# sacs-epfl/decentralized-learning-simulator

Measured on AMD Instinct MI355X. Metric: device-resident GB/s, N-way weighted model-tensor reduce; 1/2/4/8 MI355X, higher is better.
Workload: dtype f32

## Files before the change

decentralized-learning-simulator_amd/csrc/dispatch.hpp:

```cpp
#pragma once

#include <hip/hip_runtime.h>

#include <algorithm>
#include <cmath>
#include <cstdint>
#include <cstdlib>
#include <cstring>
#include <type_traits>
#include <vector>

#include "dlsim.h"
#include "wreduce_kernels.hpp"
#include "chunk_mean_kernels.hpp"
#include "ab_env.hpp"


namespace dlsim_host __attribute__((visibility("hidden"))) {

int fail(int code, const char* fmt, ...) __attribute__((format(printf, 2, 3)));
int hip_fail(hipError_t e, const char* what);

constexpr int kVpt = 4;
constexpr size_t kBatchSmallBytes = size_t{1} << 20;
// ... 416 lines not shown
    if (nelem[t] * Op::kBytes > kMaxLaunchOutBytes) return false;
    if (use_defer<Op>(fan_in[t], nelem[t])) return false;
    if (!aligned16(outs[t])) return false;
    for (int i = 0; i < fan_in[t]; ++i)
      if (!aligned16(in[off[t] + i])) return false;
    return true;
  };
  std::vector<int> group;
  for (int t = 0; t < b; ++t) {
    if (batchable(t)) {
      group.push_back(t);
      continue;
    }
    if (nelem[t] == 0) continue;
    int rc = run<Op>(in + off[t], fan_in[t], w + off[t], outs[t], nelem[t], st, divs ? divs[t] : 1.0f);
    if (rc != DLSIM_OK) return rc;
  }
  std::vector<const void*> ins;
  std::vector<float> ws, dv;
  std::vector<void*> os;
  std::vector<size_t> ne, ioff;
  std::vector<int> fi;
  for (int t : group) {
    ioff.push_back(ins.size());
    for (int i = 0; i < fan_in[t]; ++i) {
      ins.push_back(in[off[t] + i]);
      ws.push_back(w[off[t] + i]);
    }
    os.push_back(outs[t]);
    ne.push_back(nelem[t]);
    fi.push_back(fan_in[t]);
    dv.push_back(divs ? divs[t] : 1.0f);
  }
  const int g = static_cast<int>(group.size());
  const size_t tile1 = dlsim::kBlock;
  int t0 = 0;
  while (t0 < g) {
    int t1 = t0, ptrs = 0;
    uint64_t blocks = 0;
    while (t1 < g && t1 - t0 < dlsim::kBatchMaxTasks && ptrs + fi[t1] <= dlsim::kBatchMaxPtrs &&
           blocks + ne[t1] / Op::E / tile1 + 1 < 0x7fffffffull) {
      ptrs += fi[t1];
      blocks += ne[t1] / Op::E / tile1 + 1;
      ++t1;
    }
    hipError_t e = launch_batch<Op>(fi.data(), ioff.data(), ins.data(), ws.data(), dv.data(), os.data(),
                                    ne.data(), t0, t1, st);
    if (e != hipSuccess) return hip_fail(e, "batched kernel launch");
    t0 = t1;
  }
  return DLSIM_OK;
}

struct TableLayout {
  size_t tasks_off, map_off, ptrs_off, w_off, bytes;
  uint32_t nblocks;
  int vpt;
};

inline size_t round8(size_t x) { return (x + 7) / 8 * 8; }

template <class Op>
uint32_t task_blocks(size_t nelem, int vpt) {
  const size_t tile = static_cast<size_t>(dlsim::kBlock) * vpt;
  return static_cast<uint32_t>(nelem / Op::E / tile + 1);
}

template <class Op>
bool table_layout(int b, const int* fan_in, const size_t* nelem, TableLayout* L) {
  uint64_t blocks = 0, ptrs = 0;
  L->vpt = batch_vpt<Op>(nelem, 0, b);
  for (int t = 0; t < b; ++t) {
    blocks += task_blocks<Op>(nelem[t], L->vpt);
    ptrs += static_cast<uint64_t>(fan_in[t]);
  }
  if (blocks >= 0x7fffffffull) return false;
  L->nblocks = static_cast<uint32_t>(blocks);
  L->tasks_off = round8(sizeof(dlsim::BatchTableHeader));
  L->map_off = round8(L->tasks_off + sizeof(dlsim::BatchTaskDesc) * static_cast<size_t>(b));
  L->ptrs_off = round8(L->map_off + sizeof(uint32_t) * static_cast<size_t>(blocks));
  L->w_off = round8(L->ptrs_off + sizeof(void*) * static_cast<size_t>(ptrs));
  L->bytes = round8(L->w_off + sizeof(float) * static_cast<size_t>(ptrs));
  return true;
}

template <class Op>
int table_fill(int b, const int* fan_in, const void* const* in, const float* w, void* const* outs,
               const size_t* nelem, void* h_table, size_t bytes) {
  TableLayout L;
  if (!table_layout<Op>(b, fan_in, nelem, &L)) return fail(DLSIM_E_ARG, "batch too large");
  if (bytes < L.bytes) return fail(DLSIM_E_ARG, "table buffer too small (%zu < %zu)", bytes, L.bytes);
  if (cross_task_overlap(b, fan_in, in, outs, nelem, Op::kBytes))
    return fail(DLSIM_E_ARG,
                "a task's output overlaps another task's input or output: one table launch runs all tasks "
                "concurrently (use separate calls, or dlsim_wreduce_batched, which orders them)");
  unsigned char* base = static_cast<unsigned char*>(h_table);
  std::memset(base, 0, L.bytes);
  auto* h = reinterpret_cast<dlsim::BatchTableHeader*>(base);
  auto* tasks = reinterpret_cast<dlsim::BatchTaskDesc*>(base + L.tasks_off);
  auto* map = reinterpret_cast<uint32_t*>(base + L.map_off);
  auto* ptrs = reinterpret_cast<const void**>(base + L.ptrs_off);
  auto* ws = reinterpret_cast<float*>(base + L.w_off);
  h->ntasks = static_cast<uint32_t>(b);
  h->nblocks = L.nblocks;
  h->vpt = static_cast<uint32_t>(L.vpt);
  h->tasks_off = L.tasks_off;
  h->map_off = L.map_off;
  h->ptrs_off = L.ptrs_off;
  h->w_off = L.w_off;
  uint32_t blk = static_cast<uint32_t>(b), off = 0;
  bool uniform = true;
  for (int t = 0; t < b; ++t) {
    const size_t total = nelem[t] * Op::kBytes;
    if (fan_in[t] > DLSIM_MAX_FUSED_INPUTS || total > kMaxLaunchOutBytes || !aligned16(outs[t]))
      return fail(DLSIM_E_ARG, "task %d cannot be table-batched (fan-in <= %d, 16-B aligned, < 2 GiB)", t,
                  DLSIM_MAX_FUSED_INPUTS);
    const uint32_t nb = task_blocks<Op>(nelem[t], L.vpt);
    tasks[t].out = outs[t];
    tasks[t].nvec = nelem[t] / Op::E;
    tasks[t].nelem = nelem[t];
    tasks[t].block_start = blk - 1;
    tasks[t].ptr_off = off;
    tasks[t].fan_in = static_cast<uint32_t>(fan_in[t]);
    map[t] = static_cast<uint32_t>(t);
    for (uint32_t k = 0; k + 1 < nb; ++k) map[blk + k] = static_cast<uint32_t>(t);
    for (int i = 0; i < fan_in[t]; ++i) {
      if (!aligned16(in[off + i]))
        return fail(DLSIM_E_ARG, "task %d input %d is not 16-byte aligned", t, i);
      ptrs[off + i] = in[off + i];
      ws[off + i] = w[off + i];
    }
    blk += nb - 1;
    off += static_cast<uint32_t>(fan_in[t]);
    uniform = uniform && fan_in[t] == fan_in[0];
  }
  h->uniform_fan_in = uniform ? static_cast<uint32_t>(fan_in[0]) : 0u;
  return DLSIM_OK;
}

template <class Op, int NF, int VPT>
hipError_t launch_table_nf(const void* d_table, uint32_t blocks, hipStream_t st) {
  hipLaunchKernelGGL((dlsim::k_wreduce_batch_table<Op, NF, group_size<Op>(), VPT, kNT, store_policy<Op>(),
                                                    kBatchWave<Op, VPT>>),
                     dim3(blocks), dim3(dlsim::kBlock), 0, st, static_cast<const unsigned char*>(d_table));
  return hipGetLastError();
}

template <class Op, int K, int VPT>
hipError_t launch_table_fixed(const void* d_table, int n, uint32_t blocks, hipStream_t st) {
  if constexpr (K > max_fixed_fan_in<Op>()) {
    return launch_table_nf<Op, 0, VPT>(d_table, blocks, st);
  } else {
    if (n == K) return launch_table_nf<Op, K, VPT>(d_table, blocks, st);
    return launch_table_fixed<Op, K + 1, VPT>(d_table, n, blocks, st);
  }
}

template <class Op>
int table_launch(const void* h_table, const void* d_table, hipStream_t st) {
  const auto* h = static_cast<const dlsim::BatchTableHeader*>(h_table);
  if (h->ntasks == 0) return DLSIM_OK;
  if (h->vpt != 1 && h->vpt != 4)
    return fail(DLSIM_E_ARG, "not a table written by dlsim_batch_table_fill (vectors per lane %u)", h->vpt);
  const int n = static_cast<int>(h->uniform_fan_in);
  hipError_t e;
  if (h->vpt == 1)
    e = n ? launch_table_fixed<Op, 1, 1>(d_table, n, h->nblocks, st) : launch_table_nf<Op, 0, 1>(d_table, h->nblocks, st);
  else
    e = n ? launch_table_fixed<Op, 1, 4>(d_table, n, h->nblocks, st) : launch_table_nf<Op, 0, 4>(d_table, h->nblocks, st);
  if (e != hipSuccess) return hip_fail(e, "table batch launch");
  return DLSIM_OK;
}


inline size_t chunk_mean_ilp_begin(int m, size_t n, int threads, size_t esz = 4, size_t vw = 8) {
  if (n <= 1) return 0;
  const size_t rnd = 128 / esz;
  size_t b = 0, e = n;
  if (!(static_cast<unsigned long long>(m) * n < 32768ULL || threads <= 1)) {
    const size_t tp = static_cast<size_t>(threads) < n ? static_cast<size_t>(threads) : n;
    const size_t cs = (n + tp - 1) / tp;
    for (size_t t = 0; t < tp; ++t) {
      size_t tb = t * cs;
      if (tb >= n) break;
      size_t te = tb + cs < n ? tb + cs : n;
      tb -= tb % rnd;
      if (te != n) te -= te % rnd;
      if (tb < te) {
        b = tb;
        e = te;
      }
    }
  }
  const size_t s1 = e - b;
  return b + (s1 >= vw ? s1 / (4 * vw) * (4 * vw) : s1 / 4 * 4);
}

using CmDefault = dlsim::CmShape<4, true, 8>;
using CmFewRows = dlsim::CmShape<4, true, 4>;
constexpr int kCmFewRowsMax = 6;

constexpr int kCmDeferRMax = 32, kCmDeferU = kDeferU, kCmDeferMinRows = 16;
inline bool chunk_defer_on() {
  static const bool on = [] {
    const char* e = dlsim::ab_getenv("DLSIM_CHUNK_DEFER");
    return !(e && e[0] == '0');
  }();
  return on;
}
inline int chunk_defer_min_m() {
  static const int k = [] {
    const char* e = dlsim::ab_getenv("DLSIM_CHUNK_DEFER_MIN_M");
    return e ? std::atoi(e) : kCmDeferMinRows;
  }();
  return k;
}
constexpr int kCmFixedMinM = 4, kCmFixedMaxM = 15;
inline bool chunk_defer_fixed_on() {
  static const bool on = [] {
    const char* e = dlsim::ab_getenv("DLSIM_CHUNK_DEFER_FIXED");
    return !(e && e[0] == '0');
  }();
  return on;
// ... 157 lines not shown
                         dim3(dlsim::kBlock), 0, st, s);
    }
    hipError_t e = hipGetLastError();
    if (e != hipSuccess) return hip_fail(e, "chunk mean batch launch");
    batch.clear();
    np = 0;
    tiles = 0;
    return DLSIM_OK;
  };
  for (int t = 0; t < b; ++t) {
    const size_t n = nelem[t];
    if (n == 0) continue;
    const int m = fan_in[t];
    const size_t ib = chunk_mean_ilp_begin(m, n, threads, Op::kBytes == 8 ? 8 : 4, dlsim::cm_lanes<Op>());
    const uint8_t flags = task_flags(t);
    const uint32_t head = m > dlsim::kCmMaxPtrs ? 0u : task_head(t, ib, flags);
    const size_t tb = task_blocks(ib, head);
    if (m > dlsim::kCmMaxPtrs) {
      void* d = nullptr;
      const size_t bytes = static_cast<size_t>(m) * sizeof(void*);
      hipError_t e = hipMallocAsync(&d, bytes, st);
      if (e != hipSuccess) return hip_fail(e, "chunk mean pointer table alloc");
      e = hipMemcpyAsync(d, in + off[t], bytes, hipMemcpyHostToDevice, st);
      if (e == hipSuccess) {
        hipLaunchKernelGGL((dlsim::k_chunk_mean_table<Op, CmDefault>), dim3(static_cast<unsigned>(tb)),
                           dim3(dlsim::kBlock), 0, st, static_cast<const void* const*>(d), m, outs[t], n, ib,
                           flags);
        e = hipGetLastError();
      }
      hipError_t e2 = hipFreeAsync(d, st);
      if (e != hipSuccess) return hip_fail(e, "chunk mean table launch");
      if (e2 != hipSuccess) return hip_fail(e2, "chunk mean pointer table free");
      continue;
    }
    if (static_cast<int>(batch.size()) == dlsim::kCmMaxTasks || np + m > dlsim::kCmMaxPtrs ||
        tiles + tb > 0x7fffffffu) {
      int rc = flush();
      if (rc != DLSIM_OK) return rc;
    }
    batch.push_back({t, ib, flags, head});
    np += m;
    tiles += tb;
  }
  return flush();
}

}

#define DLSIM_REDUCE_ENTRIES(X, Op)                                                                      \
  X int dlsim_host::run<Op>(const void* const*, int, const float*, void*, size_t, hipStream_t, float);  \
  X int dlsim_host::run_batched<Op>(int, const int*, const void* const*, const float*, void* const*,    \
                                    const size_t*, hipStream_t, const float*);                          \
  X bool dlsim_host::table_layout<Op>(int, const int*, const size_t*, dlsim_host::TableLayout*);        \
  X int dlsim_host::table_fill<Op>(int, const int*, const void* const*, const float*, void* const*,     \
                                   const size_t*, void*, size_t);                                       \
  X int dlsim_host::table_launch<Op>(const void*, const void*, hipStream_t);
#define DLSIM_MEAN_ENTRIES(X, Op)                                                                        \
  X int dlsim_host::run<Op>(const void* const*, int, const float*, void*, size_t, hipStream_t, float);  \
  X int dlsim_host::run_batched<Op>(int, const int*, const void* const*, const float*, void* const*,    \
                                    const size_t*, hipStream_t, const float*);                          \
  X int dlsim_host::run_chunk_mean<Op>(int, const int*, const void* const*, void* const*, const size_t*, \
                                       int, hipStream_t);
#define DLSIM_PROBE_ENTRIES(X, Op) \
  X int dlsim_host::run<Op>(const void* const*, int, const float*, void*, size_t, hipStream_t, float);
#define DLSIM_F64_ENTRIES(X, Op) \
  X int dlsim_host::run<Op>(const void* const*, int, const double*, void*, size_t, hipStream_t, float);
#define DLSIM_CHUNK_ENTRIES(X, Op)                                                                       \
  X int dlsim_host::run_chunk_mean<Op>(int, const int*, const void* const*, void* const*, const size_t*, \
                                       int, hipStream_t);

#define DLSIM_ALL_ENTRIES(X)                  \
  DLSIM_REDUCE_ENTRIES(X, dlsim::F32Exact)    \
  DLSIM_REDUCE_ENTRIES(X, dlsim::F32Fast)     \
  DLSIM_REDUCE_ENTRIES(X, dlsim::BF16Exact)   \
  DLSIM_REDUCE_ENTRIES(X, dlsim::BF16Fast)    \
  DLSIM_REDUCE_ENTRIES(X, dlsim::F16Exact)    \
  DLSIM_REDUCE_ENTRIES(X, dlsim::F16Fast)     \
  DLSIM_MEAN_ENTRIES(X, dlsim::F32Mean)       \
  DLSIM_MEAN_ENTRIES(X, dlsim::BF16Mean)      \
  DLSIM_MEAN_ENTRIES(X, dlsim::F16Mean)       \
  DLSIM_PROBE_ENTRIES(X, dlsim::XorProbe<4>)  \
  DLSIM_PROBE_ENTRIES(X, dlsim::XorProbe<2>)  \
  DLSIM_F64_ENTRIES(X, dlsim::F64Exact)       \
  DLSIM_F64_ENTRIES(X, dlsim::F64Fast)        \
  DLSIM_CHUNK_ENTRIES(X, dlsim::F64Mean)
```

decentralized-learning-simulator_amd/csrc/dlsim_abi.hip:

```cpp
#include <hip/hip_runtime.h>

#include <algorithm>
#include <cstdarg>
#include <cstdio>
#include <cstdint>
#include <cstdlib>
#include <cstring>
#include <mutex>
#include <string>
#include <thread>
#include <vector>

#include "abi_common.hpp"
#include "dispatch.hpp"
#include "fanin_checks.hpp"

#include "host_pack.hpp"

namespace dlsim_host __attribute__((visibility("hidden"))) {

template <class F>
int with_policy(int dtype, int mode, F&& f) {
  const bool fast = mode == DLSIM_FAST;
  if (dtype == DLSIM_F32) return fast ? f(dlsim::F32Fast{}) : f(dlsim::F32Exact{});
// ... 317 lines not shown
int dlsim_wreduce_tensors(const void* const* d_inputs, int n, int t, const size_t* numels,
                          const float* h_weights, void* const* d_outs, int dtype, int mode,
                          void* stream) {
  g_err.clear();
  if (t < 0) return fail(DLSIM_E_ARG, "t must be >= 0 (got %d)", t);
  if (t > 0 && (!d_inputs || !numels || !d_outs)) return fail(DLSIM_E_ARG, "null array argument");
  if (n < 1) return fail(DLSIM_E_ARG, "n must be >= 1 (got %d)", n);
  if (!h_weights) return fail(DLSIM_E_ARG, "null weights array");
  std::vector<const void*> ins(static_cast<size_t>(n) * t);
  std::vector<float> ws(static_cast<size_t>(n) * t);
  std::vector<int> fan(static_cast<size_t>(t), n);
  for (int k = 0; k < t; ++k) {
    for (int i = 0; i < n; ++i) {
      ins[static_cast<size_t>(k) * n + i] = d_inputs[static_cast<size_t>(i) * t + k];
      ws[static_cast<size_t>(k) * n + i] = h_weights[i];
    }
    int rc = check_args(&ins[static_cast<size_t>(k) * n], n, h_weights, d_outs[k], numels[k], dtype, mode);
    if (rc != DLSIM_OK) return fail(rc, "tensor %d: %s", k, g_err.c_str());
  }
  if (t == 0) return DLSIM_OK;
  hipStream_t st = static_cast<hipStream_t>(stream);
  return with_policy(dtype, mode, [&](auto op) {
    return run_batched<decltype(op)>(t, fan.data(), ins.data(), ws.data(), d_outs, numels, st);
  });
}

int dlsim_wreduce_batched(int b, const int* fan_in, const void* const* d_inputs,
                          const float* h_weights, void* const* d_outs, const size_t* n_elems,
                          int dtype, int mode, void* stream) {
  g_err.clear();
  if (b < 0) return fail(DLSIM_E_ARG, "b must be >= 0 (got %d)", b);
  if (b == 0) return DLSIM_OK;
  if (!fan_in || !d_inputs || !h_weights || !d_outs || !n_elems) return fail(DLSIM_E_ARG, "null array argument");
  size_t off = 0;
  for (int t = 0; t < b; ++t) {
    int rc = check_args(d_inputs + off, fan_in[t], h_weights + off, d_outs[t], n_elems[t], dtype, mode);
    if (rc != DLSIM_OK) return fail(rc, "task %d: %s", t, g_err.c_str());
    off += static_cast<size_t>(fan_in[t]);
  }
  hipStream_t st = static_cast<hipStream_t>(stream);
  return with_policy(dtype, mode, [&](auto op) {
    return run_batched<decltype(op)>(b, fan_in, d_inputs, h_weights, d_outs, n_elems, st);
  });
}

int dlsim_batch_table_bytes(int b, const int* fan_in, const size_t* n_elems, int dtype, size_t* bytes) {
  g_err.clear();
  if (b < 0 || (b > 0 && (!fan_in || !n_elems)) || !bytes) return fail(DLSIM_E_ARG, "bad arguments");
  if (!known_dtype(dtype)) return dtype_fail(dtype);
  for (int t = 0; t < b; ++t)
    if (fan_in[t] < 1) return fail(DLSIM_E_ARG, "task %d: fan-in must be >= 1", t);
  TableLayout L;
  const bool ok = with_policy(dtype, DLSIM_EXACT, [&](auto op) {
    return table_layout<decltype(op)>(b, fan_in, n_elems, &L) ? 1 : 0;
  }) != 0;
  if (!ok) return fail(DLSIM_E_ARG, "batch too large");
  *bytes = L.bytes;
  return DLSIM_OK;
}

int dlsim_batch_table_fill(int b, const int* fan_in, const void* const* d_inputs, const float* h_weights,
                           void* const* d_outs, const size_t* n_elems, int dtype, void* h_table,
                           size_t table_bytes) {
  g_err.clear();
  if (b < 0 || !h_table) return fail(DLSIM_E_ARG, "bad arguments");
  if (b > 0 && (!fan_in || !d_inputs || !h_weights || !d_outs || !n_elems))
    return fail(DLSIM_E_ARG, "null array argument");
  size_t off = 0;
  for (int t = 0; t < b; ++t) {
    int rc = check_args(d_inputs + off, fan_in[t], h_weights + off, d_outs[t], n_elems[t], dtype, DLSIM_EXACT);
    if (rc != DLSIM_OK) return fail(rc, "task %d: %s", t, g_err.c_str());
    off += static_cast<size_t>(fan_in[t]);
  }
  return with_policy(dtype, DLSIM_EXACT, [&](auto op) {
    return table_fill<decltype(op)>(b, fan_in, d_inputs, h_weights, d_outs, n_elems, h_table, table_bytes);
  });
}

int dlsim_batch_table_launch(const void* h_table, const void* d_table, int dtype, int mode, void* stream) {
  g_err.clear();
  if (!h_table || !d_table) return fail(DLSIM_E_ARG, "null table");
  if (!known_dtype(dtype)) return dtype_fail(dtype);
  if (mode != DLSIM_EXACT && mode != DLSIM_FAST) return fail(DLSIM_E_MODE, "unsupported mode %d", mode);
  hipStream_t st = static_cast<hipStream_t>(stream);
  return with_policy(dtype, mode, [&](auto op) { return table_launch<decltype(op)>(h_table, d_table, st); });
}

int dlsim_mean(const void* const* d_inputs, int n, void* d_out, size_t n_elems, int dtype,
               void* stream) {
  g_err.clear();
  int rc = check_args(d_inputs, n, nullptr, d_out, n_elems, dtype, DLSIM_EXACT, false);
  if (rc != DLSIM_OK) return rc;
  hipStream_t st = static_cast<hipStream_t>(stream);
  const float div = static_cast<float>(n);
  return with_mean_policy(dtype, [&](auto op) {
    return run<decltype(op)>(d_inputs, n, nullptr, d_out, n_elems, st, div);
  });
}

int dlsim_mean_batched(int b, const int* fan_in, const void* const* d_inputs, void* const* d_outs,
                       const size_t* n_elems, int dtype, void* stream) {
  g_err.clear();
  if (b < 0) return fail(DLSIM_E_ARG, "b must be >= 0 (got %d)", b);
  if (b == 0) return DLSIM_OK;
  if (!fan_in || !d_inputs || !d_outs || !n_elems) return fail(DLSIM_E_ARG, "null array argument");
  size_t off = 0;
  std::vector<float> divs(static_cast<size_t>(b));
  for (int t = 0; t < b; ++t) {
    int rc = check_args(d_inputs + off, fan_in[t], nullptr, d_outs[t], n_elems[t], dtype, DLSIM_EXACT, false);
    if (rc != DLSIM_OK) return fail(rc, "task %d: %s", t, g_err.c_str());
// ... 932 lines not shown
```

decentralized-learning-simulator_amd/csrc/wreduce_kernels.hpp:

```cpp
#pragma once

#include <hip/hip_runtime.h>
#include <stdint.h>

#include <type_traits>

#pragma clang fp contract(off)

namespace dlsim {

constexpr int kBlock = 256;

typedef uint32_t u32x4 __attribute__((ext_vector_type(4)));
typedef float f32x2 __attribute__((ext_vector_type(2)));
typedef __bf16 bf16x2 __attribute__((ext_vector_type(2)));

__device__ __forceinline__ float bf16_round(float f) {
  uint32_t u = __float_as_uint(f);
  if ((u & 0x7fffffffu) > 0x7f800000u) return __uint_as_float(0x7fc00000u);
  u += 0x7fffu + ((u >> 16) & 1u);
  return __uint_as_float(u & 0xffff0000u);
}

__device__ __forceinline__ void bf16_round2(float& a0, float& a1) {
// ... 724 lines not shown
}

struct TaskArgs {
  const BatchSlots& b;
  int off;
  float d;
  __device__ const void* ptr(int i) const { return b.p[off + i]; }
  __device__ float wt(int i) const { return b.w[off + i]; }
  __device__ float divisor() const { return d; }
};

template <class Op, int NF, int G, int VPT, int NT, int STP, bool WAVEMAP = false>
__global__ __launch_bounds__(kBlock) void k_wreduce_batch(const BatchSlots s) {
  const uint32_t bid = blockIdx.x;
  int t = 0;
  uint32_t local = 0;
  if (bid < static_cast<uint32_t>(s.ntasks)) {
    t = static_cast<int>(bid);
  } else {
    const uint32_t f = bid - static_cast<uint32_t>(s.ntasks);
    t = batch_find_task(s, f);
    local = f - s.block_start[t] + 1;
  }
  const TaskArgs a{s, static_cast<int>(s.ptr_off[t]), s.div[t]};
  const int n = NF > 0 ? NF : static_cast<int>(s.fan_in[t]);
  const size_t nvec = s.nvec[t];
  constexpr size_t kTile = static_cast<size_t>(kBlock) * VPT;
  const size_t full = nvec / kTile;
  const OutRef o = make_out<STP>(s.out[t], nvec);
  if (local == 0) {
    if (full * kTile < nvec)
      reduce_tile<Op, TaskArgs, NF, G, VPT, NT, true, STP>(a, n, o, full * kTile + threadIdx.x, nvec);
    const size_t j = nvec * Op::E + threadIdx.x;
    if (j < s.nelem[t]) fold_scalar<Op, TaskArgs>(a, n, s.out[t], j);
    return;
  }
  if constexpr (WAVEMAP) {
    const size_t lane_off = (threadIdx.x >> 6) * 64 * VPT + (threadIdx.x & 63);
    reduce_tile<Op, TaskArgs, NF, G, VPT, NT, false, STP, 64>(a, n, o, (local - 1) * kTile + lane_off, nvec);
  } else {
    reduce_tile<Op, TaskArgs, NF, G, VPT, NT, false, STP>(a, n, o, (local - 1) * kTile + threadIdx.x, nvec);
  }
}

struct BatchTableHeader {
  uint32_t ntasks;
  uint32_t nblocks;
  uint32_t uniform_fan_in;
  uint32_t vpt;
  uint64_t tasks_off;
  uint64_t map_off;
  uint64_t ptrs_off;
  uint64_t w_off;
};

struct BatchTaskDesc {
  void* out;
  uint64_t nvec;
  uint64_t nelem;
  uint32_t block_start;
  uint32_t ptr_off;
  uint32_t fan_in;
  uint32_t reserved;
};

struct TableArgs {
  const void* const* p;
  const float* w;
  __device__ const void* ptr(int i) const { return p[i]; }
  __device__ float wt(int i) const { return w[i]; }
  __device__ float divisor() const { return 1.0f; }
};

template <class Op, int NF, int G, int VPT, int NT, int STP, bool WAVEMAP = false>
__global__ __launch_bounds__(kBlock) void k_wreduce_batch_table(const unsigned char* __restrict__ table) {
  const BatchTableHeader* h = reinterpret_cast<const BatchTableHeader*>(table);
  const uint32_t* map = reinterpret_cast<const uint32_t*>(table + h->map_off);
  const uint32_t t = map[blockIdx.x];
  const BatchTaskDesc d = reinterpret_cast<const BatchTaskDesc*>(table + h->tasks_off)[t];
  const TableArgs a{reinterpret_cast<const void* const*>(table + h->ptrs_off) + d.ptr_off,
                    reinterpret_cast<const float*>(table + h->w_off) + d.ptr_off};
  const int n = NF > 0 ? NF : static_cast<int>(d.fan_in);
  const size_t nvec = d.nvec;
  constexpr size_t kTile = static_cast<size_t>(kBlock) * VPT;
  const size_t full = nvec / kTile;
  const OutRef o = make_out<STP>(d.out, nvec);
  const uint32_t local = blockIdx.x < h->ntasks ? 0u : blockIdx.x - d.block_start;
  if (local == 0) {
    if (full * kTile < nvec)
      reduce_tile<Op, TableArgs, NF, G, VPT, NT, true, STP>(a, n, o, full * kTile + threadIdx.x, nvec);
    const size_t j = nvec * Op::E + threadIdx.x;
    if (j < d.nelem) fold_scalar<Op, TableArgs>(a, n, d.out, j);
    return;
  }
  if constexpr (WAVEMAP) {
    const size_t lane_off = (threadIdx.x >> 6) * 64 * VPT + (threadIdx.x & 63);
    reduce_tile<Op, TableArgs, NF, G, VPT, NT, false, STP, 64>(a, n, o, (local - 1) * kTile + lane_off, nvec);
  } else {
    reduce_tile<Op, TableArgs, NF, G, VPT, NT, false, STP>(a, n, o, (local - 1) * kTile + threadIdx.x, nvec);
  }
}

template <int BYTES>
struct XorProbe {
  static constexpr int E = 16 / BYTES;
  static constexpr int kBytes = BYTES;
// ... 87 lines not shown
```

decentralized-learning-simulator_amd/dasklearn_amd/_native.py:

```python
from __future__ import annotations

import ctypes
import os
import threading
from typing import Optional, Sequence

import numpy as np

LIB_DIR = os.path.join(os.path.dirname(os.path.abspath(__file__)), "lib")
LIB_PATH = os.path.join(LIB_DIR, "libdlsim_hip.so")

DLSIM_F32 = 0
DLSIM_BF16 = 1
DLSIM_F16 = 2
DLSIM_F64 = 3
DLSIM_EXACT = 0
DLSIM_FAST = 1
MAX_FUSED_INPUTS = 128
DLSIM_E_ARG = -1
DLSIM_E_RCCL = -4
DLSIM_E_PEER = -5
DLSIM_E_DISAGREE = -6
DLSIM_GATHER_NONE = 0
DLSIM_GATHER_BCAST = 1
DLSIM_GATHER_ALLGATHER = 2


def ab_env(name: str, default: Optional[str] = None) -> Optional[str]:
    if os.environ.get("DLSIM_AB") != "1":
        return default
    return os.environ.get(name, default)

EXPORTS = (
    "dlsim_wreduce",
    "dlsim_wreduce_f64",
    "dlsim_wreduce_tensors",
    "dlsim_wreduce_batched",
    "dlsim_batch_table_bytes",
    "dlsim_batch_table_fill",
    "dlsim_batch_table_launch",
    "dlsim_mean",
    "dlsim_mean_batched",
    "dlsim_chunk_mean_batched",
    "dlsim_chunk_mean_ilp_begin",
    "dlsim_rccl_bind",
    "dlsim_wreduce_sharded",
    "dlsim_wreduce_sharded_f64",
    "dlsim_wreduce_mixed",
    "dlsim_sgd_step",
    "dlsim_sgd_step_tensors",
    "dlsim_sgd_momentum_step",
    "dlsim_sgd_momentum_step_tensors",
    "dlsim_robust_reduce",
    "dlsim_robust_reduce_tensors",
    "dlsim_robust_reduce_batched",
    "dlsim_robust_batch_geometry",
    "dlsim_robust_reduce_tensors_batched",
    "dlsim_pairwise_sqdist",
    "dlsim_pairwise_sqdist_tensors",
    "dlsim_pairdist_geometry",
    "dlsim_wreduce_dist",
    "dlsim_wreduce_dist_tensors",
    "dlsim_reducedist_geometry",
    "dlsim_device_alloc",
    "dlsim_device_free",
    "dlsim_pool_alloc",
    "dlsim_pool_free",
    "dlsim_pool_stats",
    "dlsim_sharded_plan_create",
    "dlsim_sharded_plan_run",
    "dlsim_sharded_plan_run_f64",
    "dlsim_sharded_plan_destroy",
    "dlsim_host_wreduce",
    "dlsim_host_wreduce_zc",
    "dlsim_host_wreduce_resident",
    "dlsim_host_chunk_mean",
    "dlsim_host_pack",
    "dlsim_shard_range",
    "dlsim_probe_pattern",
    "dlsim_kernel_name",
    "dlsim_last_error",
    "dlsim_version",
)

_lib = None
_lock = threading.Lock()


class DlsimError(RuntimeError):

    def __init__(self, fn: str, rc: int, msg: str):
        super().__init__(f"{fn} failed (rc={rc}): {msg}")
        self.rc = rc


def load() -> ctypes.CDLL:
    global _lib
    if _lib is not None:
        return _lib
    with _lock:
        if _lib is not None:
            return _lib
        if not os.path.exists(LIB_PATH):
            raise ImportError(
                f"HIP extension not built: {LIB_PATH} is missing. Run "
                "`python -c 'import __graft_entry__ as g; g.build()'` at the repo root.")
        lib = ctypes.CDLL(LIB_PATH)
        vp, sz, i = ctypes.c_void_p, ctypes.c_size_t, ctypes.c_int
        lib.dlsim_wreduce.argtypes = [ctypes.POINTER(vp), i, ctypes.POINTER(ctypes.c_float), vp,
                                      sz, i, i, vp]
        lib.dlsim_wreduce.restype = i
        lib.dlsim_wreduce_f64.argtypes = [ctypes.POINTER(vp), i, ctypes.POINTER(ctypes.c_double), vp, sz, i, vp]
        lib.dlsim_wreduce_f64.restype = i
        lib.dlsim_wreduce_tensors.argtypes = [ctypes.POINTER(vp), i, i, ctypes.POINTER(sz),
                                              ctypes.POINTER(ctypes.c_float), ctypes.POINTER(vp),
                                              i, i, vp]
        lib.dlsim_wreduce_tensors.restype = i
        lib.dlsim_wreduce_batched.argtypes = [i, ctypes.POINTER(i), ctypes.POINTER(vp),
                                              ctypes.POINTER(ctypes.c_float), ctypes.POINTER(vp),
                                              ctypes.POINTER(sz), i, i, vp]
        lib.dlsim_wreduce_batched.restype = i
        lib.dlsim_batch_table_bytes.argtypes = [i, ctypes.POINTER(i), ctypes.POINTER(sz), i,
                                                ctypes.POINTER(sz)]
        lib.dlsim_batch_table_bytes.restype = i
        lib.dlsim_batch_table_fill.argtypes = [i, ctypes.POINTER(i), ctypes.POINTER(vp),
                                               ctypes.POINTER(ctypes.c_float), ctypes.POINTER(vp),
                                               ctypes.POINTER(sz), i, vp, sz]
        lib.dlsim_batch_table_fill.restype = i
        lib.dlsim_batch_table_launch.argtypes = [vp, vp, i, i, vp]
        lib.dlsim_batch_table_launch.restype = i
        lib.dlsim_mean.argtypes = [ctypes.POINTER(vp), i, vp, sz, i, vp]
        lib.dlsim_mean.restype = i
        lib.dlsim_mean_batched.argtypes = [i, ctypes.POINTER(i), ctypes.POINTER(vp), ctypes.POINTER(vp),
                                           ctypes.POINTER(sz), i, vp]
        lib.dlsim_mean_batched.restype = i
        lib.dlsim_chunk_mean_batched.argtypes = [i, ctypes.POINTER(i), ctypes.POINTER(vp), ctypes.POINTER(vp),
                                                 ctypes.POINTER(sz), i, i, vp]
        lib.dlsim_chunk_mean_batched.restype = i
        lib.dlsim_chunk_mean_ilp_begin.argtypes = [i, sz, i]
        lib.dlsim_chunk_mean_ilp_begin.restype = sz
        lib.dlsim_rccl_bind.argtypes = [ctypes.c_char_p]
        lib.dlsim_rccl_bind.restype = i
        lib.dlsim_wreduce_sharded.argtypes = [ctypes.POINTER(vp), sz, i, ctypes.POINTER(ctypes.c_float), vp, sz, i,
                                              i, vp, i, vp]
        lib.dlsim_wreduce_sharded.restype = i
        lib.dlsim_wreduce_sharded_f64.argtypes = [ctypes.POINTER(vp), sz, i, ctypes.POINTER(ctypes.c_double), vp,
                                                  sz, i, vp, i, vp]
        lib.dlsim_wreduce_sharded_f64.restype = i
        lib.dlsim_sharded_plan_create.argtypes = [vp, sz, i, i, i, vp, ctypes.POINTER(vp)]
        lib.dlsim_sharded_plan_create.restype = i
        lib.dlsim_sharded_plan_run.argtypes = [vp, ctypes.POINTER(vp), sz, ctypes.POINTER(ctypes.c_float), vp, i, vp]
        lib.dlsim_sharded_plan_run.restype = i
        lib.dlsim_sharded_plan_run_f64.argtypes = [vp, ctypes.POINTER(vp), sz, ctypes.POINTER(ctypes.c_double), vp,
                                                   i, vp]
        lib.dlsim_sharded_plan_run_f64.restype = i
        lib.dlsim_sharded_plan_destroy.argtypes = [vp]
        lib.dlsim_sharded_plan_destroy.restype = i
        lib.dlsim_host_wreduce.argtypes = [i, i, ctypes.POINTER(vp), ctypes.POINTER(sz),
                                           ctypes.POINTER(ctypes.c_float), vp, vp, sz, vp, vp, i, i, sz, i,
                                           vp, vp, vp]
        lib.dlsim_host_wreduce.restype = i
        lib.dlsim_host_wreduce_zc.argtypes = [i, i, ctypes.POINTER(vp), ctypes.POINTER(sz),
                                              ctypes.POINTER(ctypes.c_float), vp, sz, vp, i, i, i, vp]
        lib.dlsim_host_wreduce_zc.restype = i
        lib.dlsim_host_wreduce_resident.argtypes = [i, i, ctypes.POINTER(vp), ctypes.POINTER(sz),
                                                    ctypes.POINTER(ctypes.c_float), ctypes.POINTER(i),
                                                    ctypes.POINTER(vp), vp, sz, vp, vp, i, i, i, vp]
        lib.dlsim_host_wreduce_resident.restype = i
        lib.dlsim_host_chunk_mean.argtypes = [i, ctypes.POINTER(i), ctypes.POINTER(vp), ctypes.POINTER(sz), vp, vp,
                                              sz, ctypes.POINTER(vp), ctypes.POINTER(vp), i, i, i, vp, vp, vp]
        lib.dlsim_host_chunk_mean.restype = i
        lib.dlsim_host_pack.argtypes = [i, ctypes.POINTER(vp), ctypes.POINTER(sz), ctypes.POINTER(sz), vp, i]
        lib.dlsim_host_pack.restype = i
        lib.dlsim_shard_range.argtypes = [sz, i, i, sz, ctypes.POINTER(sz), ctypes.POINTER(sz)]
        lib.dlsim_shard_range.restype = i
        lib.dlsim_probe_pattern.argtypes = [ctypes.POINTER(vp), i, vp, sz, i, vp]
        lib.dlsim_probe_pattern.restype = i
        lib.dlsim_wreduce_mixed.argtypes = [ctypes.POINTER(vp), ctypes.POINTER(i), i, ctypes.POINTER(ctypes.c_double),
                                            vp, i, sz, vp]
        lib.dlsim_wreduce_mixed.restype = i
        lib.dlsim_sgd_step.argtypes = [vp, vp, vp, sz, ctypes.c_double, ctypes.c_double, i, vp]
        lib.dlsim_sgd_step.restype = i
        lib.dlsim_sgd_step_tensors.argtypes = [i, ctypes.POINTER(vp), ctypes.POINTER(vp), ctypes.POINTER(vp),
# ... 494 lines not shown
                with torch.cuda.device(self.device_index):
                    _lib.dlsim_device_free(ptr)
            except Exception:
                pass


def wreduce(inputs, weights_f32, out, mode: int = DLSIM_EXACT, stream=None):
    ReducePlan(inputs, weights_f32, out, mode).launch(stream)
    return out


class BatchPlan:

    def __init__(self, tasks, mode: int = DLSIM_EXACT):
        import torch
        self.b = len(tasks)
        out0 = tasks[0][2]
        self.device, self.mode, self.dtype = out0.device, mode, dtype_code(out0.dtype)
        fan, ptrs, ws, outs, numels = [], [], [], [], []
        for inputs, w32, out in tasks:
            if len(w32) != len(inputs):
                raise AssertionError("weights/models length mismatch")
            for t in list(inputs) + [out]:
                if not t.is_cuda or t.dtype != out0.dtype or t.numel() != out.numel() \
                        or not t.is_contiguous() or t.device != self.device:
                    raise ValueError("each task: contiguous device tensors of one dtype, size and device")
            fan.append(len(inputs))
            ptrs.extend(t.data_ptr() for t in inputs)
            ws.extend(np.asarray(w32, dtype=np.float32).tolist())
            outs.append(out.data_ptr())
            numels.append(out.numel())
        lib = load()
        c_fan = (ctypes.c_int * self.b)(*fan)
        c_num = (ctypes.c_size_t * self.b)(*numels)
        nbytes = ctypes.c_size_t(0)
        _check("dlsim_batch_table_bytes",
               lib.dlsim_batch_table_bytes(self.b, c_fan, c_num, self.dtype, ctypes.byref(nbytes)))
        self._h = torch.empty(nbytes.value, dtype=torch.uint8, pin_memory=True)
        _check("dlsim_batch_table_fill",
               lib.dlsim_batch_table_fill(self.b, c_fan, (ctypes.c_void_p * len(ptrs))(*ptrs),
                                          (ctypes.c_float * len(ws))(*ws),
                                          (ctypes.c_void_p * self.b)(*outs), c_num, self.dtype,
                                          self._h.data_ptr(), nbytes.value))
        self._d = self._h.to(self.device, non_blocking=True)
        torch.cuda.current_stream(self.device).synchronize()
        self._keep = tasks
        self._lib = lib

    def launch(self, stream=None) -> None:
        _check("dlsim_batch_table_launch",
               self._lib.dlsim_batch_table_launch(self._h.data_ptr(), self._d.data_ptr(), self.dtype,
                                                  self.mode, _stream_handle(self.device, stream)))


def wreduce_batched(tasks, mode: int = DLSIM_EXACT, stream=None):
    lib = load()
    b = len(tasks)
    if b == 0:
        return []
    dt = dtype_code(tasks[0][2].dtype)
    fan, ptrs, ws, outs, numels = [], [], [], [], []
    for inputs, w32, out in tasks:
        if len(inputs) < 1:
            raise IndexError("list index out of range")
        if len(w32) != len(inputs):
            raise AssertionError("weights/models length mismatch")
        for t in list(inputs) + [out]:
            if not t.is_cuda or t.dtype != out.dtype or t.numel() != out.numel() or not t.is_contiguous() \
                    or t.device != out.device:
                raise ValueError("each task: contiguous device tensors of one dtype, size and device")
        if out.dtype != tasks[0][2].dtype or out.device != tasks[0][2].device:
            raise ValueError("all tasks of a batch share dtype and device")
        fan.append(len(inputs))
        ptrs.extend(t.data_ptr() for t in inputs)
        ws.extend(np.asarray(w32, dtype=np.float32).tolist())
        outs.append(out.data_ptr())
        numels.append(out.numel())
    c_fan = (ctypes.c_int * b)(*fan)
    c_ptrs = (ctypes.c_void_p * len(ptrs))(*ptrs)
    c_w = (ctypes.c_float * len(ws))(*ws)
    c_outs = (ctypes.c_void_p * b)(*outs)
    c_num = (ctypes.c_size_t * b)(*numels)
    _check("dlsim_wreduce_batched",
           lib.dlsim_wreduce_batched(b, c_fan, c_ptrs, c_w, c_outs, c_num, dt, mode,
                                     _stream_handle(tasks[0][2].device, stream)))
    return [t[2] for t in tasks]


def mean(inputs, out, stream=None):
    lib = load()
    n = len(inputs)
    if n < 1:
        raise IndexError("list index out of range")
    dt = dtype_code(out.dtype)
    for t in list(inputs) + [out]:
        if not t.is_cuda or t.dtype != out.dtype or t.numel() != out.numel() or not t.is_contiguous() \
                or t.device != out.device:
            raise ValueError("inputs and output must be contiguous tensors of one dtype and size "
                             "on one device")
    ptrs = (ctypes.c_void_p * n)(*[t.data_ptr() for t in inputs])
    _check("dlsim_mean", lib.dlsim_mean(ptrs, n, out.data_ptr(), out.numel(), dt,
                                        _stream_handle(out.device, stream)))
    return out


def mean_batched(tasks, stream=None):
# ... 483 lines not shown
```

include/dlsim.h:

```cpp
#ifndef DLSIM_H_
#define DLSIM_H_

#include <stddef.h>
#include <stdint.h>

#ifdef __cplusplus
extern "C" {
#endif

enum dlsim_dtype {
  DLSIM_F32 = 0,
  DLSIM_BF16 = 1,
  DLSIM_F16 = 2,
  DLSIM_F64 = 3
};

enum dlsim_mode {
  DLSIM_EXACT = 0,
  DLSIM_FAST = 1
};

#define DLSIM_OK 0
#define DLSIM_E_ARG (-1)
#define DLSIM_E_DTYPE (-2)
#define DLSIM_E_MODE (-3)
#define DLSIM_E_RCCL (-4)
#define DLSIM_E_PEER (-5)
#define DLSIM_E_DISAGREE (-6)

enum dlsim_gather {
  DLSIM_GATHER_NONE = 0,
  DLSIM_GATHER_BCAST = 1,
  DLSIM_GATHER_ALLGATHER = 2
};
#define DLSIM_E_HIP (-100)

#define DLSIM_MAX_FUSED_INPUTS 128

int dlsim_wreduce(const void* const* d_inputs, int n, const float* h_weights,
                  void* d_out, size_t n_elems, int dtype, int mode,
                  void* stream);

int dlsim_wreduce_f64(const void* const* d_inputs, int n, const double* h_weights, void* d_out, size_t n_elems,
                      int mode, void* stream);

int dlsim_wreduce_tensors(const void* const* d_inputs, int n, int t,
                          const size_t* numels, const float* h_weights,
                          void* const* d_outs, int dtype, int mode,
                          void* stream);

int dlsim_wreduce_batched(int b, const int* fan_in, const void* const* d_inputs,
                          const float* h_weights, void* const* d_outs, const size_t* n_elems,
                          int dtype, int mode, void* stream);

int dlsim_batch_table_bytes(int b, const int* fan_in, const size_t* n_elems, int dtype,
                            size_t* bytes);
int dlsim_batch_table_fill(int b, const int* fan_in, const void* const* d_inputs,
                           const float* h_weights, void* const* d_outs, const size_t* n_elems,
                           int dtype, void* h_table, size_t table_bytes);
int dlsim_batch_table_launch(const void* h_table, const void* d_table, int dtype, int mode,
                             void* stream);

int dlsim_mean(const void* const* d_inputs, int n, void* d_out, size_t n_elems, int dtype,
               void* stream);

int dlsim_mean_batched(int b, const int* fan_in, const void* const* d_inputs, void* const* d_outs,
                       const size_t* n_elems, int dtype, void* stream);

int dlsim_chunk_mean_batched(int b, const int* fan_in, const void* const* d_inputs, void* const* d_outs,
                             const size_t* n_elems, int dtype, int cpu_threads, void* stream);

size_t dlsim_chunk_mean_ilp_begin(int m, size_t n_elems, int cpu_threads);

int dlsim_rccl_bind(const char* librccl_path);

int dlsim_wreduce_sharded(const void* const* d_slices, size_t slice_elems, int n, const float* h_weights,
                          void* d_out, size_t n_elems, int dtype, int mode, void* rccl_comm, int gather,
                          void* stream);

int dlsim_wreduce_sharded_f64(const void* const* d_slices, size_t slice_elems, int n, const double* h_weights,
                              void* d_out, size_t n_elems, int mode, void* rccl_comm, int gather, void* stream);

typedef struct dlsim_sharded_plan dlsim_sharded_plan;

int dlsim_sharded_plan_create(void* rccl_comm, size_t n_elems, int n, int dtype, int gather, void* stream,
                              dlsim_sharded_plan** plan);
int dlsim_sharded_plan_run(dlsim_sharded_plan* plan, const void* const* d_slices, size_t slice_elems,
                           const float* h_weights, void* d_out, int mode, void* stream);
int dlsim_sharded_plan_run_f64(dlsim_sharded_plan* plan, const void* const* d_slices, size_t slice_elems,
                               const double* h_weights, void* d_out, int mode, void* stream);
int dlsim_sharded_plan_destroy(dlsim_sharded_plan* plan);

int dlsim_host_wreduce(int n, int t, const void* const* h_srcs, const size_t* numels,
                       const float* h_weights, void* h_staging, void* d_rows, size_t row_stride,
                       void* d_out, void* h_out, int dtype, int mode, size_t chunk_elems, int threads,
                       void* stream, void* h2d_stream, void* d2h_stream);

int dlsim_host_wreduce_zc(int n, int t, const void* const* h_srcs, const size_t* numels, const float* h_weights,
                          void* h_staging, size_t row_stride, void* h_out, int dtype, int mode, int threads,
                          void* stream);

int dlsim_host_wreduce_resident(int n, int t, const void* const* h_srcs, const size_t* numels,
                                const float* h_weights, const int* resident, void* const* d_rows, void* h_staging,
                                size_t staging_stride, void* d_out, void* h_out, int dtype, int mode, int threads,
                                void* stream);

int dlsim_host_chunk_mean(int b, const int* fan_in, const void* const* h_inputs, const size_t* n_elems,
                          void* h_staging, void* d_staging, size_t staging_elems, void* const* d_outs,
                          void* const* h_outs, int dtype, int cpu_threads, int threads, void* stream,
// ... 86 lines not shown
```

Baseline: 6621.

## Run large table-batch tasks as standalone launches instead of inside the fused table kernel

Table fill now sorts tasks into two groups. Tasks at or above a size threshold (about 11 MB, overridable by environment variable) that qualify for the deferred path go to the end of the task list and launch one by one through the regular run path. Smaller tasks stay in the fused table kernel, with vectors-per-lane chosen only from the tasks that remain. This aims to give big tensors the tuned single-task kernels while small tasks keep the batching, at the cost of extra launches and a larger table-size bound.

```diff
diff --git a/decentralized-learning-simulator_amd/csrc/dispatch.hpp b/decentralized-learning-simulator_amd/csrc/dispatch.hpp
--- a/decentralized-learning-simulator_amd/csrc/dispatch.hpp
+++ b/decentralized-learning-simulator_amd/csrc/dispatch.hpp
@@ -492,10 +492,20 @@
   return DLSIM_OK;
 }
 
+constexpr double kTableAloneMinMB = 11.18;
+inline double table_alone_min_mb() {
+  static const double x = [] {
+    const char* e = dlsim::ab_getenv("DLSIM_TABLE_ALONE_MIN_MB");
+    return e ? std::atof(e) : kTableAloneMinMB;
+  }();
+  return x;
+}
+
 struct TableLayout {
   size_t tasks_off, map_off, ptrs_off, w_off, bytes;
   uint32_t nblocks;
   int vpt;
+  int stay;
 };
 
 inline size_t round8(size_t x) { return (x + 7) / 8 * 8; }
@@ -507,74 +517,114 @@
 }
 
 template <class Op>
-bool table_layout(int b, const int* fan_in, const size_t* nelem, TableLayout* L) {
-  uint64_t blocks = 0, ptrs = 0;
-  L->vpt = batch_vpt<Op>(nelem, 0, b);
-  for (int t = 0; t < b; ++t) {
-    blocks += task_blocks<Op>(nelem[t], L->vpt);
-    ptrs += static_cast<uint64_t>(fan_in[t]);
-  }
-  if (blocks >= 0x7fffffffull) return false;
+bool table_alone(int n, size_t nelem) {
+  const size_t bytes = nelem * Op::kBytes;
+  return n <= DLSIM_MAX_FUSED_INPUTS && bytes <= kMaxLaunchOutBytes &&
+         static_cast<double>(bytes) >= table_alone_min_mb() * 1e6 && use_defer<Op>(n, nelem);
+}
+
+inline void table_offsets(int b, uint64_t blocks, uint64_t ptrs, TableLayout* L) {
   L->nblocks = static_cast<uint32_t>(blocks);
   L->tasks_off = round8(sizeof(dlsim::BatchTableHeader));
   L->map_off = round8(L->tasks_off + sizeof(dlsim::BatchTaskDesc) * static_cast<size_t>(b));
   L->ptrs_off = round8(L->map_off + sizeof(uint32_t) * static_cast<size_t>(blocks));
   L->w_off = round8(L->ptrs_off + sizeof(void*) * static_cast<size_t>(ptrs));
   L->bytes = round8(L->w_off + sizeof(float) * static_cast<size_t>(ptrs));
+}
+
+template <class Op>
+bool table_bound(int b, const int* fan_in, const size_t* nelem, TableLayout* L) {
+  uint64_t blocks = 0, ptrs = 0;
+  for (int t = 0; t < b; ++t) {
+    blocks += task_blocks<Op>(nelem[t], batch_vpt<Op>(nelem, t, t + 1));
+    ptrs += static_cast<uint64_t>(fan_in[t]);
+  }
+  if (blocks >= 0x7fffffffull) return false;
+  L->vpt = 0;
+  L->stay = b;
+  table_offsets(b, blocks, ptrs, L);
+  return true;
+}
+
+template <class Op>
+bool table_layout(int b, const int* fan_in, const size_t* nelem, TableLayout* L) {
+  uint64_t blocks = 0, ptrs = 0;
+  size_t mx = 0;
+  L->stay = 0;
+  for (int t = 0; t < b; ++t) {
+    ptrs += static_cast<uint64_t>(fan_in[t]);
+    if (table_alone<Op>(fan_in[t], nelem[t])) continue;
+    mx = std::max(mx, nelem[t]);
+    ++L->stay;
+  }
+  L->vpt = batch_vpt<Op>(&mx, 0, 1);
+  for (int t = 0; t < b; ++t)
+    if (!table_alone<Op>(fan_in[t], nelem[t])) blocks += task_blocks<Op>(nelem[t], L->vpt);
+  if (blocks >= 0x7fffffffull) return false;
+  table_offsets(b, blocks, ptrs, L);
   return true;
 }
 
 template <class Op>
 int table_fill(int b, const int* fan_in, const void* const* in, const float* w, void* const* outs,
                const size_t* nelem, void* h_table, size_t bytes) {
-  TableLayout L;
-  if (!table_layout<Op>(b, fan_in, nelem, &L)) return fail(DLSIM_E_ARG, "batch too large");
-  if (bytes < L.bytes) return fail(DLSIM_E_ARG, "table buffer too small (%zu < %zu)", bytes, L.bytes);
+  TableLayout L, bound;
+  if (!table_bound<Op>(b, fan_in, nelem, &bound) || !table_layout<Op>(b, fan_in, nelem, &L))
+    return fail(DLSIM_E_ARG, "batch too large");
+  if (bytes < bound.bytes || bound.bytes < L.bytes)
+    return fail(DLSIM_E_ARG, "table buffer too small (%zu < %zu)", bytes, std::max(bound.bytes, L.bytes));
   if (cross_task_overlap(b, fan_in, in, outs, nelem, Op::kBytes))
     return fail(DLSIM_E_ARG,
                 "a task's output overlaps another task's input or output: one table launch runs all tasks "
                 "concurrently (use separate calls, or dlsim_wreduce_batched, which orders them)");
   unsigned char* base = static_cast<unsigned char*>(h_table);
-  std::memset(base, 0, L.bytes);
+  std::memset(base, 0, bound.bytes);
   auto* h = reinterpret_cast<dlsim::BatchTableHeader*>(base);
   auto* tasks = reinterpret_cast<dlsim::BatchTaskDesc*>(base + L.tasks_off);
   auto* map = reinterpret_cast<uint32_t*>(base + L.map_off);
   auto* ptrs = reinterpret_cast<const void**>(base + L.ptrs_off);
   auto* ws = reinterpret_cast<float*>(base + L.w_off);
-  h->ntasks = static_cast<uint32_t>(b);
+  h->ntasks = static_cast<uint32_t>(L.stay);
   h->nblocks = L.nblocks;
   h->vpt = static_cast<uint32_t>(L.vpt);
   h->tasks_off = L.tasks_off;
   h->map_off = L.map_off;
   h->ptrs_off = L.ptrs_off;
   h->w_off = L.w_off;
-  uint32_t blk = static_cast<uint32_t>(b), off = 0;
+  h->total_tasks = static_cast<uint32_t>(b);
+  h->nalone = static_cast<uint32_t>(b - L.stay);
+  uint32_t blk = static_cast<uint32_t>(L.stay), off = 0;
+  int stay = 0, alone = L.stay, fan0 = 0;
   bool uniform = true;
   for (int t = 0; t < b; ++t) {
     const size_t total = nelem[t] * Op::kBytes;
     if (fan_in[t] > DLSIM_MAX_FUSED_INPUTS || total > kMaxLaunchOutBytes || !aligned16(outs[t]))
       return fail(DLSIM_E_ARG, "task %d cannot be table-batched (fan-in <= %d, 16-B aligned, < 2 GiB)", t,
                   DLSIM_MAX_FUSED_INPUTS);
-    const uint32_t nb = task_blocks<Op>(nelem[t], L.vpt);
-    tasks[t].out = outs[t];
-    tasks[t].nvec = nelem[t] / Op::E;
-    tasks[t].nelem = nelem[t];
-    tasks[t].block_start = blk - 1;
-    tasks[t].ptr_off = off;
-    tasks[t].fan_in = static_cast<uint32_t>(fan_in[t]);
-    map[t] = static_cast<uint32_t>(t);
-    for (uint32_t k = 0; k + 1 < nb; ++k) map[blk + k] = static_cast<uint32_t>(t);
+    const bool leaves = table_alone<Op>(fan_in[t], nelem[t]);
+    const int slot = leaves ? alone++ : stay++;
+    tasks[slot].out = outs[t];
+    tasks[slot].nvec = nelem[t] / Op::E;
+    tasks[slot].nelem = nelem[t];
+    tasks[slot].ptr_off = off;
+    tasks[slot].fan_in = static_cast<uint32_t>(fan_in[t]);
     for (int i = 0; i < fan_in[t]; ++i) {
       if (!aligned16(in[off + i]))
         return fail(DLSIM_E_ARG, "task %d input %d is not 16-byte aligned", t, i);
       ptrs[off + i] = in[off + i];
       ws[off + i] = w[off + i];
     }
+    off += static_cast<uint32_t>(fan_in[t]);
+    if (leaves) continue;
+    const uint32_t nb = task_blocks<Op>(nelem[t], L.vpt);
+    tasks[slot].block_start = blk - 1;
+    map[slot] = static_cast<uint32_t>(slot);
+    for (uint32_t k = 0; k + 1 < nb; ++k) map[blk + k] = static_cast<uint32_t>(slot);
     blk += nb - 1;
-    off += static_cast<uint32_t>(fan_in[t]);
-    uniform = uniform && fan_in[t] == fan_in[0];
-  }
-  h->uniform_fan_in = uniform ? static_cast<uint32_t>(fan_in[0]) : 0u;
+    if (slot == 0) fan0 = fan_in[t];
+    uniform = uniform && fan_in[t] == fan0;
+  }
+  h->uniform_fan_in = uniform ? static_cast<uint32_t>(fan0) : 0u;
   return DLSIM_OK;
 }
 
@@ -596,19 +646,43 @@
   }
 }
 
+inline bool table_split(const void* h_table, int* in_table_kernel, int* alone) {
+  const auto* h = static_cast<const dlsim::BatchTableHeader*>(h_table);
+  if (h->ntasks > 0x7fffffffu || h->nalone > 0x7fffffffu || h->ntasks + h->nalone != h->total_tasks) return false;
+  if (in_table_kernel) *in_table_kernel = static_cast<int>(h->ntasks);
+  if (alone) *alone = static_cast<int>(h->nalone);
+  return true;
+}
+
+inline const dlsim::BatchTaskDesc* table_tasks(const dlsim::BatchTableHeader* h) {
+  return reinterpret_cast<const dlsim::BatchTaskDesc*>(reinterpret_cast<const unsigned char*>(h) + h->tasks_off);
+}
+
 template <class Op>
 int table_launch(const void* h_table, const void* d_table, hipStream_t st) {
   const auto* h = static_cast<const dlsim::BatchTableHeader*>(h_table);
-  if (h->ntasks == 0) return DLSIM_OK;
-  if (h->vpt != 1 && h->vpt != 4)
-    return fail(DLSIM_E_ARG, "not a table written by dlsim_batch_table_fill (vectors per lane %u)", h->vpt);
-  const int n = static_cast<int>(h->uniform_fan_in);
-  hipError_t e;
-  if (h->vpt == 1)
-    e = n ? launch_table_fixed<Op, 1, 1>(d_table, n, h->nblocks, st) : launch_table_nf<Op, 0, 1>(d_table, h->nblocks, st);
-  else
-    e = n ? launch_table_fixed<Op, 1, 4>(d_table, n, h->nblocks, st) : launch_table_nf<Op, 0, 4>(d_table, h->nblocks, st);
-  if (e != hipSuccess) return hip_fail(e, "table batch launch");
+  if (h->total_tasks == 0) return DLSIM_OK;
+  if ((h->vpt != 1 && h->vpt != 4) || h->ntasks + h->nalone != h->total_tasks || (h->ntasks == 0) != (h->nblocks == 0))
+    return fail(DLSIM_E_ARG, "not a table written by dlsim_batch_table_fill (vectors per lane %u, %u + %u of %u tasks)",
+                h->vpt, h->ntasks, h->nalone, h->total_tasks);
+  if (h->nblocks > 0) {
+    const int n = static_cast<int>(h->uniform_fan_in);
+    hipError_t e;
+    if (h->vpt == 1)
+      e = n ? launch_table_fixed<Op, 1, 1>(d_table, n, h->nblocks, st) : launch_table_nf<Op, 0, 1>(d_table, h->nblocks, st);
+    else
+      e = n ? launch_table_fixed<Op, 1, 4>(d_table, n, h->nblocks, st) : launch_table_nf<Op, 0, 4>(d_table, h->nblocks, st);
+    if (e != hipSuccess) return hip_fail(e, "table batch launch");
+  }
+  const unsigned char* base = static_cast<const unsigned char*>(h_table);
+  const dlsim::BatchTaskDesc* tasks = table_tasks(h);
+  const auto* ptrs = reinterpret_cast<const void* const*>(base + h->ptrs_off);
+  const auto* ws = reinterpret_cast<const float*>(base + h->w_off);
+  for (uint32_t k = h->ntasks; k < h->total_tasks; ++k) {
+    const dlsim::BatchTaskDesc& d = tasks[k];
+    int rc = run<Op>(ptrs + d.ptr_off, static_cast<int>(d.fan_in), ws + d.ptr_off, d.out, d.nelem, st);
+    if (rc != DLSIM_OK) return rc;
+  }
   return DLSIM_OK;
 }
 
@@ -872,6 +946,7 @@
   X int dlsim_host::run_batched<Op>(int, const int*, const void* const*, const float*, void* const*,    \
                                     const size_t*, hipStream_t, const float*);                          \
   X bool dlsim_host::table_layout<Op>(int, const int*, const size_t*, dlsim_host::TableLayout*);        \
+  X bool dlsim_host::table_bound<Op>(int, const int*, const size_t*, dlsim_host::TableLayout*);         \
   X int dlsim_host::table_fill<Op>(int, const int*, const void* const*, const float*, void* const*,     \
                                    const size_t*, void*, size_t);                                       \
   X int dlsim_host::table_launch<Op>(const void*, const void*, hipStream_t);
diff --git a/decentralized-learning-simulator_amd/csrc/dlsim_abi.hip b/decentralized-learning-simulator_amd/csrc/dlsim_abi.hip
--- a/decentralized-learning-simulator_amd/csrc/dlsim_abi.hip
+++ b/decentralized-learning-simulator_amd/csrc/dlsim_abi.hip
@@ -393,10 +393,18 @@
     if (fan_in[t] < 1) return fail(DLSIM_E_ARG, "task %d: fan-in must be >= 1", t);
   TableLayout L;
   const bool ok = with_policy(dtype, DLSIM_EXACT, [&](auto op) {
-    return table_layout<decltype(op)>(b, fan_in, n_elems, &L) ? 1 : 0;
+    return table_bound<decltype(op)>(b, fan_in, n_elems, &L) ? 1 : 0;
   }) != 0;
   if (!ok) return fail(DLSIM_E_ARG, "batch too large");
   *bytes = L.bytes;
+  return DLSIM_OK;
+}
+
+int dlsim_batch_table_split(const void* h_table, int* in_table_kernel, int* alone) {
+  g_err.clear();
+  if (!h_table) return fail(DLSIM_E_ARG, "null table");
+  if (!table_split(h_table, in_table_kernel, alone))
+    return fail(DLSIM_E_ARG, "not a table written by dlsim_batch_table_fill");
   return DLSIM_OK;
 }
 
diff --git a/decentralized-learning-simulator_amd/csrc/wreduce_kernels.hpp b/decentralized-learning-simulator_amd/csrc/wreduce_kernels.hpp
--- a/decentralized-learning-simulator_amd/csrc/wreduce_kernels.hpp
+++ b/decentralized-learning-simulator_amd/csrc/wreduce_kernels.hpp
@@ -800,6 +800,8 @@
   uint64_t map_off;
   uint64_t ptrs_off;
   uint64_t w_off;
+  uint32_t total_tasks;
+  uint32_t nalone;
 };
 
 struct BatchTaskDesc {
diff --git a/decentralized-learning-simulator_amd/dasklearn_amd/_native.py b/decentralized-learning-simulator_amd/dasklearn_amd/_native.py
--- a/decentralized-learning-simulator_amd/dasklearn_amd/_native.py
+++ b/decentralized-learning-simulator_amd/dasklearn_amd/_native.py
@@ -39,6 +39,7 @@
     "dlsim_batch_table_bytes",
     "dlsim_batch_table_fill",
     "dlsim_batch_table_launch",
+    "dlsim_batch_table_split",
     "dlsim_mean",
     "dlsim_mean_batched",
     "dlsim_chunk_mean_batched",
@@ -129,6 +130,8 @@
         lib.dlsim_batch_table_fill.restype = i
         lib.dlsim_batch_table_launch.argtypes = [vp, vp, i, i, vp]
         lib.dlsim_batch_table_launch.restype = i
+        lib.dlsim_batch_table_split.argtypes = [vp, ctypes.POINTER(i), ctypes.POINTER(i)]
+        lib.dlsim_batch_table_split.restype = i
         lib.dlsim_mean.argtypes = [ctypes.POINTER(vp), i, vp, sz, i, vp]
         lib.dlsim_mean.restype = i
         lib.dlsim_mean_batched.argtypes = [i, ctypes.POINTER(i), ctypes.POINTER(vp), ctypes.POINTER(vp),
@@ -729,6 +732,12 @@
                self._lib.dlsim_batch_table_launch(self._h.data_ptr(), self._d.data_ptr(), self.dtype,
                                                   self.mode, _stream_handle(self.device, stream)))
 
+    def split(self):
+        stay, alone = ctypes.c_int(0), ctypes.c_int(0)
+        _check("dlsim_batch_table_split",
+               self._lib.dlsim_batch_table_split(self._h.data_ptr(), ctypes.byref(stay), ctypes.byref(alone)))
+        return stay.value, alone.value
+
 
 def wreduce_batched(tasks, mode: int = DLSIM_EXACT, stream=None):
     lib = load()
diff --git a/include/dlsim.h b/include/dlsim.h
--- a/include/dlsim.h
+++ b/include/dlsim.h
@@ -55,6 +55,7 @@
 
 int dlsim_batch_table_bytes(int b, const int* fan_in, const size_t* n_elems, int dtype,
                             size_t* bytes);
+int dlsim_batch_table_split(const void* h_table, int* in_table_kernel, int* alone);
 int dlsim_batch_table_fill(int b, const int* fan_in, const void* const* d_inputs,
                            const float* h_weights, void* const* d_outs, const size_t* n_elems,
                            int dtype, void* h_table, size_t table_bytes);
```

Measured after the change: 6637, median of 3. Within noise of the previous version (+0.2%).
